# advimman/lama

Hardware: NVIDIA H100
Metric: images/sec FFCResNetGenerator @512x512 bs32 (higher is better)
Workload: dtype bf16x3(f32 accumulate)

## Files before the change

### lama_b200/csrc/conv_tc.cu

```cuda
#include <cuda.h>
#include <stdlib.h>

#include <type_traits>

#include "common.cuh"

namespace ffcb {
namespace {

constexpr int BM = 128;
constexpr int BK = 64;
constexpr int WG_K = 16;
constexpr int kThreads = 384;
constexpr int kConsumers = 256;
constexpr int kTileABytes = BM * BK * 2;
constexpr int kMaxStages = 8;
constexpr int kBarBytes = 1024;
constexpr int kSmemLimit = 227 * 1024;

struct TcParams {
  View out, addend;
  const float* shift;
  int N, act, addend_post;
  int BN, num_n_tiles;
  long long num_m_tiles;
  int stages;
  int flat;
  int TW, TH, tiles_x, tiles_y;
  int stride;
  int coord_off[2];
  int nseg;
  int a_il[2];
  const unsigned short* a_ptr[2];
  long long a_sg[2], a_lo[2];
  int a_tiles_per_image[2];
  int out_planar;
  int ring;
  int hints;
  int rr_dy0, rr_a_bytes, rr_w_bytes;
  int halo_a_bytes;
  signed char seg_taps[FFCB_MAX_KSEG];
  ffcb_kseg seg[FFCB_MAX_KSEG];
};

__device__ __forceinline__ uint32_t smem_u32(const void* p) { return (uint32_t)__cvta_generic_to_shared(p); }

__device__ __forceinline__ void mbar_init(uint64_t* bar, uint32_t count) {
  asm volatile("mbarrier.init.shared::cta.b64 [%0], %1;" ::"r"(smem_u32(bar)), "r"(count));
}
__device__ __forceinline__ void mbar_expect_tx(uint64_t* bar, uint32_t bytes) {
  asm volatile("mbarrier.arrive.expect_tx.shared::cta.b64 _, [%0], %1;" ::"r"(smem_u32(bar)), "r"(bytes) : "memory");
}
__device__ __forceinline__ void mbar_arrive(uint64_t* bar) {
  asm volatile("mbarrier.arrive.shared::cta.b64 _, [%0];" ::"r"(smem_u32(bar)) : "memory");
}
__device__ __forceinline__ void mbar_wait(uint64_t* bar, uint32_t parity) {
  asm volatile(
      "{\n\t"
      ".reg .pred p;\n\t"
      "WAIT_LOOP:\n\t"
      "mbarrier.try_wait.parity.shared::cta.b64 p, [%0], %1;\n\t"
      "@p bra WAIT_DONE;\n\t"
      "bra WAIT_LOOP;\n\t"
      "WAIT_DONE:\n\t"
      "}\n" ::"r"(smem_u32(bar)), "r"(parity)
      : "memory");
}

__device__ __forceinline__ void tma_load_3d(void* dst, const CUtensorMap* map, uint64_t* bar, int c0, int c1, int c2) {
  asm volatile(
      "cp.async.bulk.tensor.3d.shared::cluster.global.mbarrier::complete_tx::bytes [%0], [%1, {%3, %4, %5}], [%2];"
      ::"r"(smem_u32(dst)), "l"(map), "r"(smem_u32(bar)), "r"(c0), "r"(c1), "r"(c2)
      : "memory");
}
__device__ __forceinline__ void tma_load_5d(void* dst, const CUtensorMap* map, uint64_t* bar, int c0, int c1, int c2,
                                            int c3, int c4) {
  asm volatile(
      "cp.async.bulk.tensor.5d.shared::cluster.global.mbarrier::complete_tx::bytes [%0], [%1, {%3, %4, %5, %6, %7}], [%2];"
      ::"r"(smem_u32(dst)), "l"(map), "r"(smem_u32(bar)), "r"(c0), "r"(c1), "r"(c2), "r"(c3), "r"(c4)
      : "memory");
}

__device__ __forceinline__ void bulk_load(void* dst, const void* src, uint32_t bytes, uint64_t* bar) {
  asm volatile("cp.async.bulk.shared::cluster.global.mbarrier::complete_tx::bytes [%0], [%1], %2, [%3];"
               ::"r"(smem_u32(dst)), "l"(src), "r"(bytes), "r"(smem_u32(bar)) : "memory");
}

__device__ __forceinline__ void prefetch_tmap(const CUtensorMap* map) {
  asm volatile("prefetch.tensormap [%0];" ::"l"(map) : "memory");
}

constexpr uint32_t kLoSw = 1u << 16;
constexpr uint32_t kHiSw = (uint32_t)(1024 >> 4) | (1u << 30);
constexpr uint32_t kLoIl = (uint32_t)(2048 >> 4) << 16;
constexpr uint32_t kHiIl = (uint32_t)(128 >> 4);

__device__ __forceinline__ uint32_t desc_addr(uint32_t saddr) { return (saddr & 0x3FFFF) >> 4; }

__device__ __forceinline__ uint64_t desc64(uint32_t lo, uint32_t hi) {
  uint64_t d;
  asm("mov.b64 %0, {%1, %2};" : "=l"(d) : "r"(lo), "r"(hi));
  return d;
}
__device__ __forceinline__ bool elect_one() {
  uint32_t pred;
  asm volatile(
      "{\n\t"
      ".reg .pred P;\n\t"
      "elect.sync _|P, 0xffffffff;\n\t"
      "selp.b32 %0, 1, 0, P;\n\t"
      "}\n"
      : "=r"(pred));
  return pred != 0;
}

__device__ __forceinline__ void wgmma_fence() { asm volatile("wgmma.fence.sync.aligned;" ::: "memory"); }
__device__ __forceinline__ void wgmma_commit() { asm volatile("wgmma.commit_group.sync.aligned;" ::: "memory"); }
template <int N>
__device__ __forceinline__ void wgmma_wait() { asm volatile("wgmma.wait_group.sync.aligned %0;" ::"n"(N) : "memory"); }
template <int BN>
__device__ __forceinline__ void fence_acc(float* d) {
#pragma unroll
  for (int i = 0; i < BN / 2; ++i) asm volatile("" : "+f"(d[i])::"memory");
}

__device__ __forceinline__ void wgmma_n32(float* d, uint64_t da, uint64_t db, uint32_t scale_d) {
  asm volatile(
      "{\n\t.reg .pred p;\n\tsetp.ne.b32 p, %18, 0;\n\t"
      "wgmma.mma_async.sync.aligned.m64n32k16.f32.bf16.bf16 {"
      "%0, %1, %2, %3, %4, %5, %6, %7, %8, %9, %10, %11, %12, %13, %14, %15"
      "}, %16, %17, p, 1, 1, 0, 0;\n\t}\n"
      : "+f"(d[0]), "+f"(d[1]), "+f"(d[2]), "+f"(d[3]), "+f"(d[4]), "+f"(d[5]), "+f"(d[6]), "+f"(d[7]),
        "+f"(d[8]), "+f"(d[9]), "+f"(d[10]), "+f"(d[11]), "+f"(d[12]), "+f"(d[13]), "+f"(d[14]), "+f"(d[15])
      : "l"(da), "l"(db), "r"(scale_d));
}
__device__ __forceinline__ void wgmma_n64(float* d, uint64_t da, uint64_t db, uint32_t scale_d) {
  asm volatile(
      "{\n\t.reg .pred p;\n\tsetp.ne.b32 p, %34, 0;\n\t"
      "wgmma.mma_async.sync.aligned.m64n64k16.f32.bf16.bf16 {"
      "%0, %1, %2, %3, %4, %5, %6, %7, %8, %9, %10, %11, %12, %13, %14, %15, "
      "%16, %17, %18, %19, %20, %21, %22, %23, %24, %25, %26, %27, %28, %29, %30, %31"
      "}, %32, %33, p, 1, 1, 0, 0;\n\t}\n"
      : "+f"(d[0]), "+f"(d[1]), "+f"(d[2]), "+f"(d[3]), "+f"(d[4]), "+f"(d[5]), "+f"(d[6]), "+f"(d[7]),
        "+f"(d[8]), "+f"(d[9]), "+f"(d[10]), "+f"(d[11]), "+f"(d[12]), "+f"(d[13]), "+f"(d[14]), "+f"(d[15]),
        "+f"(d[16]), "+f"(d[17]), "+f"(d[18]), "+f"(d[19]), "+f"(d[20]), "+f"(d[21]), "+f"(d[22]), "+f"(d[23]),
        "+f"(d[24]), "+f"(d[25]), "+f"(d[26]), "+f"(d[27]), "+f"(d[28]), "+f"(d[29]), "+f"(d[30]), "+f"(d[31])
      : "l"(da), "l"(db), "r"(scale_d));
}
__device__ __forceinline__ void wgmma_n96(float* d, uint64_t da, uint64_t db, uint32_t scale_d) {
  asm volatile(
      "{\n\t.reg .pred p;\n\tsetp.ne.b32 p, %50, 0;\n\t"
      "wgmma.mma_async.sync.aligned.m64n96k16.f32.bf16.bf16 {"
      "%0, %1, %2, %3, %4, %5, %6, %7, %8, %9, %10, %11, %12, %13, %14, %15, "
      "%16, %17, %18, %19, %20, %21, %22, %23, %24, %25, %26, %27, %28, %29, %30, %31, "
      "%32, %33, %34, %35, %36, %37, %38, %39, %40, %41, %42, %43, %44, %45, %46, %47"
      "}, %48, %49, p, 1, 1, 0, 0;\n\t}\n"
      : "+f"(d[0]), "+f"(d[1]), "+f"(d[2]), "+f"(d[3]), "+f"(d[4]), "+f"(d[5]), "+f"(d[6]), "+f"(d[7]),
        "+f"(d[8]), "+f"(d[9]), "+f"(d[10]), "+f"(d[11]), "+f"(d[12]), "+f"(d[13]), "+f"(d[14]), "+f"(d[15]),
        "+f"(d[16]), "+f"(d[17]), "+f"(d[18]), "+f"(d[19]), "+f"(d[20]), "+f"(d[21]), "+f"(d[22]), "+f"(d[23]),
        "+f"(d[24]), "+f"(d[25]), "+f"(d[26]), "+f"(d[27]), "+f"(d[28]), "+f"(d[29]), "+f"(d[30]), "+f"(d[31]),
        "+f"(d[32]), "+f"(d[33]), "+f"(d[34]), "+f"(d[35]), "+f"(d[36]), "+f"(d[37]), "+f"(d[38]), "+f"(d[39]),
        "+f"(d[40]), "+f"(d[41]), "+f"(d[42]), "+f"(d[43]), "+f"(d[44]), "+f"(d[45]), "+f"(d[46]), "+f"(d[47])
      : "l"(da), "l"(db), "r"(scale_d));
}
__device__ __forceinline__ void wgmma_n128(float* d, uint64_t da, uint64_t db, uint32_t scale_d) {
  asm volatile(
      "{\n\t.reg .pred p;\n\tsetp.ne.b32 p, %66, 0;\n\t"
      "wgmma.mma_async.sync.aligned.m64n128k16.f32.bf16.bf16 {"
      "%0, %1, %2, %3, %4, %5, %6, %7, %8, %9, %10, %11, %12, %13, %14, %15, "
      "%16, %17, %18, %19, %20, %21, %22, %23, %24, %25, %26, %27, %28, %29, %30, %31, "
      "%32, %33, %34, %35, %36, %37, %38, %39, %40, %41, %42, %43, %44, %45, %46, %47, "
      "%48, %49, %50, %51, %52, %53, %54, %55, %56, %57, %58, %59, %60, %61, %62, %63"
      "}, %64, %65, p, 1, 1, 0, 0;\n\t}\n"
      : "+f"(d[0]), "+f"(d[1]), "+f"(d[2]), "+f"(d[3]), "+f"(d[4]), "+f"(d[5]), "+f"(d[6]), "+f"(d[7]),
        "+f"(d[8]), "+f"(d[9]), "+f"(d[10]), "+f"(d[11]), "+f"(d[12]), "+f"(d[13]), "+f"(d[14]), "+f"(d[15]),
        "+f"(d[16]), "+f"(d[17]), "+f"(d[18]), "+f"(d[19]), "+f"(d[20]), "+f"(d[21]), "+f"(d[22]), "+f"(d[23]),
        "+f"(d[24]), "+f"(d[25]), "+f"(d[26]), "+f"(d[27]), "+f"(d[28]), "+f"(d[29]), "+f"(d[30]), "+f"(d[31]),
        "+f"(d[32]), "+f"(d[33]), "+f"(d[34]), "+f"(d[35]), "+f"(d[36]), "+f"(d[37]), "+f"(d[38]), "+f"(d[39]),
        "+f"(d[40]), "+f"(d[41]), "+f"(d[42]), "+f"(d[43]), "+f"(d[44]), "+f"(d[45]), "+f"(d[46]), "+f"(d[47]),
        "+f"(d[48]), "+f"(d[49]), "+f"(d[50]), "+f"(d[51]), "+f"(d[52]), "+f"(d[53]), "+f"(d[54]), "+f"(d[55]),
        "+f"(d[56]), "+f"(d[57]), "+f"(d[58]), "+f"(d[59]), "+f"(d[60]), "+f"(d[61]), "+f"(d[62]), "+f"(d[63])
      : "l"(da), "l"(db), "r"(scale_d));
}
template <int BN>
__device__ __forceinline__ void wgmma_bn(float* d, uint64_t da, uint64_t db, uint32_t scale_d) {
  static_assert(BN == 32 || BN == 64 || BN == 96 || BN == 128, "N tile");
  if constexpr (BN == 32) wgmma_n32(d, da, db, scale_d);
  else if constexpr (BN == 64) wgmma_n64(d, da, db, scale_d);
  else if constexpr (BN == 96) wgmma_n96(d, da, db, scale_d);
  else wgmma_n128(d, da, db, scale_d);
}

struct TileCoord {
  int b, y0, x0;
  long long m0;
};

__device__ __forceinline__ TileCoord tile_coord(const TcParams& p, long long m_tile) {
  TileCoord t;
  if (p.flat) {
    t.m0 = m_tile * BM;
    t.b = 0; t.y0 = 0; t.x0 = 0;
  } else {
    const int per_img = p.tiles_x * p.tiles_y;
    t.b = (int)(m_tile / per_img);
    const int r = (int)(m_tile - (long long)t.b * per_img);
    t.y0 = (r / p.tiles_x) * p.TH;
    t.x0 = (r % p.tiles_x) * p.TW;
    t.m0 = 0;
  }
  return t;
}

template <bool IL, bool PO, bool RR, bool HALO, int BN>
__global__ void __launch_bounds__(kThreads, 1)
conv_tc_kernel(const __grid_constant__ TcParams p, const __grid_constant__ CUtensorMap map_in0,
               const __grid_constant__ CUtensorMap map_in1, const __grid_constant__ CUtensorMap map_w) {
  extern __shared__ __align__(1024) uint8_t smem_raw[];
  uint8_t* smem = reinterpret_cast<uint8_t*>((reinterpret_cast<uintptr_t>(smem_raw) + 1023) & ~(uintptr_t)1023);
  const int w_bytes = p.BN * BK * 2;
  const int stage_bytes = RR ? 2 * p.rr_a_bytes : HALO ? 2 * w_bytes : 2 * kTileABytes + 2 * w_bytes;
  uint8_t* w_res = smem;
  uint8_t* a_buf = smem;
  if constexpr (RR) smem += p.rr_w_bytes;
  if constexpr (HALO) smem += (size_t)4 * p.halo_a_bytes;
  uint64_t* bars = reinterpret_cast<uint64_t*>(smem + (size_t)p.stages * stage_bytes);
  uint64_t* full = bars;
  uint64_t* empty = bars + kMaxStages;
  uint64_t* w_bar = bars + 2 * kMaxStages;
  uint64_t* a_full = bars + 2 * kMaxStages + 1;
  uint64_t* a_empty = a_full + 2;

  const int warp = threadIdx.x >> 5, lane = threadIdx.x & 31;

  if (warp == 0 && lane == 0) {
    prefetch_tmap(&map_in0);
    prefetch_tmap(&map_in1);
    prefetch_tmap(&map_w);
  }
  if (warp == 1 && lane == 0) {
    for (int s = 0; s < p.stages; ++s) { mbar_init(&full[s], 1); mbar_init(&empty[s], kConsumers); }
    if constexpr (RR) mbar_init(w_bar, 1);
    if constexpr (HALO)
      for (int s = 0; s < 2; ++s) { mbar_init(&a_full[s], 1); mbar_init(&a_empty[s], kConsumers); }
    asm volatile("fence.mbarrier_init.release.cluster;" ::: "memory");
  }
  __syncthreads();

  int total_kblocks = 0;
  for (int s = 0; s < p.nseg; ++s) total_kblocks += (p.seg[s].nch + BK - 1) / BK;
  const long long num_tiles = p.num_m_tiles * p.num_n_tiles;

  if (warp == 0) {
    if constexpr (HALO) {
      int stage = 0, ast = 0;
      uint32_t phase = 0, aph = 0;
      for (long long t = blockIdx.x; t < num_tiles; t += gridDim.x) {
        const int n_tile = (int)(t % p.num_n_tiles);
        const TileCoord tc = tile_coord(p, t / p.num_n_tiles);
        int kofs = 0;
        for (int s = 0; s < p.nseg;) {
          const int ntap = p.seg_taps[s];
          const ffcb_kseg g = p.seg[s];
          const CUtensorMap* map = g.src ? &map_in1 : &map_in0;
          const int nblk = (g.nch + BK - 1) / BK;
          for (int j = 0; j < nblk; ++j) {
            for (int u = 0; u < (ntap == 9 ? 3 : 1); ++u) {
              const int dxu = ntap == 9 ? u - 1 : g.dx;
              mbar_wait(&a_empty[ast], aph ^ 1);
              if (elect_one()) {
                uint8_t* ab = a_buf + (size_t)ast * 2 * p.halo_a_bytes;
                mbar_expect_tx(&a_full[ast], 2u * p.TW * (p.TH + 2) * BK * 2);
                const int cx = tc.x0 + dxu + p.coord_off[g.src], cy = tc.y0 - 1 + p.coord_off[g.src];
                tma_load_5d(ab, map, &a_full[ast], g.c0 + j * BK, cx, cy, tc.b, 0);
                tma_load_5d(ab + p.halo_a_bytes, map, &a_full[ast], g.c0 + j * BK, cx, cy, tc.b, 1);
              }
              __syncwarp();
              if (++ast == 2) { ast = 0; aph ^= 1; }
              for (int tap = 0; tap < ntap; ++tap) {
                if (p.seg[s + tap].dx != dxu) continue;
                mbar_wait(&empty[stage], phase ^ 1);
                if (elect_one()) {
                  uint8_t* st = smem + (size_t)stage * stage_bytes;
                  mbar_expect_tx(&full[stage], (uint32_t)stage_bytes);
                  const int k = kofs + (tap * nblk + j) * BK;
                  tma_load_3d(st, &map_w, &full[stage], k, n_tile * p.BN, 0);
                  tma_load_3d(st + w_bytes, &map_w, &full[stage], k, n_tile * p.BN, 1);
                }
                __syncwarp();
                if (++stage == p.stages) { stage = 0; phase ^= 1; }
              }
            }
          }
          kofs += ntap * nblk * BK;
          s += ntap;
        }
      }
    } else if constexpr (RR) {
      const ffcb_kseg g0 = p.seg[0];
      const CUtensorMap* map = g0.src ? &map_in1 : &map_in0;
      if (elect_one()) {
        mbar_expect_tx(w_bar, (uint32_t)p.rr_w_bytes);
        for (int s = 0; s < p.nseg; ++s) {
          tma_load_3d(w_res + (size_t)s * 2 * w_bytes, &map_w, w_bar, s * BK, 0, 0);
          tma_load_3d(w_res + (size_t)s * 2 * w_bytes + w_bytes, &map_w, w_bar, s * BK, 0, 1);
        }
      }
      __syncwarp();
      int stage = 0;
      uint32_t phase = 0;
      for (long long t = blockIdx.x; t < num_tiles; t += gridDim.x) {
        const TileCoord tc = tile_coord(p, t);
        mbar_wait(&empty[stage], phase ^ 1);
        if (elect_one()) {
          uint8_t* st = smem + (size_t)stage * stage_bytes;
          mbar_expect_tx(&full[stage], (uint32_t)stage_bytes);
          const int cx = tc.x0 + g0.dx + p.coord_off[g0.src], cy = tc.y0 + p.rr_dy0 + p.coord_off[g0.src];
          tma_load_5d(st, map, &full[stage], g0.c0, cx, cy, tc.b, 0);
          tma_load_5d(st + p.rr_a_bytes, map, &full[stage], g0.c0, cx, cy, tc.b, 1);
        }
        __syncwarp();
        if (++stage == p.stages) { stage = 0; phase ^= 1; }
      }
    } else {
      int stage = 0;
      uint32_t phase = 0;
      for (long long t = blockIdx.x; t < num_tiles; t += gridDim.x) {
        const int n_tile = (int)(t % p.num_n_tiles);
        const TileCoord tc = tile_coord(p, t / p.num_n_tiles);
        int kb = 0;
        for (int s = 0; s < p.nseg; ++s) {
          const ffcb_kseg g = p.seg[s];
          const CUtensorMap* map = g.src ? &map_in1 : &map_in0;
          const int nblk = (g.nch + BK - 1) / BK;
          const int cx = tc.x0 * p.stride + g.dx + p.coord_off[g.src];
          const int cy = tc.y0 * p.stride + g.dy + p.coord_off[g.src];
          const int il = IL ? p.a_il[g.src] : 0;
          for (int j = 0; j < nblk; ++j, ++kb) {
            mbar_wait(&empty[stage], phase ^ 1);
            if (elect_one()) {
              uint8_t* st = smem + (size_t)stage * stage_bytes;
              mbar_expect_tx(&full[stage], (uint32_t)stage_bytes);
              const int cc = g.c0 + j * BK;
              if (IL && il) {
                const long long blk = p.flat ? (tc.m0 >> 7)
                                             : (long long)tc.b * p.a_tiles_per_image[g.src] + ((tc.y0 * p.out.W) >> 7);
                const unsigned short* src = p.a_ptr[g.src] + blk * p.a_sg[g.src] + (long long)(cc >> 3) * 1024;
                bulk_load(st, src, kTileABytes, &full[stage]);
                bulk_load(st + kTileABytes, src + p.a_lo[g.src], kTileABytes, &full[stage]);
              } else if (p.flat) {
                tma_load_3d(st, map, &full[stage], cc, (int)tc.m0, 0);
                tma_load_3d(st + kTileABytes, map, &full[stage], cc, (int)tc.m0, 1);
              } else {
                tma_load_5d(st, map, &full[stage], cc, cx, cy, tc.b, 0);
                tma_load_5d(st + kTileABytes, map, &full[stage], cc, cx, cy, tc.b, 1);
              }
              tma_load_3d(st + 2 * kTileABytes, &map_w, &full[stage], kb * BK, n_tile * p.BN, 0);
              tma_load_3d(st + 2 * kTileABytes + w_bytes, &map_w, &full[stage], kb * BK, n_tile * p.BN, 1);
            }
            __syncwarp();
            if (++stage == p.stages) { stage = 0; phase ^= 1; }
          }
        }
      }
    }
  } else if (warp >= 4) {
    const int g = (warp >> 2) - 1;
    const int w = warp & 3, q = lane & 3;
    const int row = g * 64 + w * 16 + (lane >> 2) + 8 * (q & 1);
    const int cb = 4 * (q >> 1);
    const bool odd = (q & 1) != 0;
    const uint32_t a_row_sw = (uint32_t)(g * 64 * BK * 2) >> 4;
    const uint32_t a_row_il = (uint32_t)(g * 64 * 16) >> 4;
    const int HW = p.out.H * p.out.W;
    const bool has_add = p.addend.ptr != nullptr;
    float acc[BN / 2];
#pragma unroll
    for (int i = 0; i < BN / 2; ++i) acc[i] = 0.f;
    int stage = 0, ast = 0;
    uint32_t phase = 0, aph = 0;
    const int a_row0 = (g + 1) * p.TW;
    if constexpr (RR) mbar_wait(w_bar, 0);
    for (long long t = blockIdx.x; t < num_tiles; t += gridDim.x) {
      const int n_tile = (int)(t % p.num_n_tiles);
      const TileCoord tc = tile_coord(p, t / p.num_n_tiles);
      fence_acc<BN>(acc);
      if constexpr (HALO) {
        int prev = -1, a_prev = -1, nt = 0;
        for (int s = 0; s < p.nseg;) {
          const int ntap = p.seg_taps[s];
          const int nblk = (p.seg[s].nch + BK - 1) / BK;
          for (int j = 0; j < nblk; ++j) {
            for (int u = 0; u < (ntap == 9 ? 3 : 1); ++u) {
              const int dxu = ntap == 9 ? u - 1 : p.seg[s].dx;
              mbar_wait(&a_full[ast], aph);
              const uint32_t ab = smem_u32(a_buf + (size_t)ast * 2 * p.halo_a_bytes);
              for (int tap = 0; tap < ntap; ++tap) {
                const int dy = p.seg[s + tap].dy;
                if (p.seg[s + tap].dx != dxu) continue;
                const uint32_t a_off = (uint32_t)((a_row0 + dy * p.TW) * (BK * 2)) >> 4;
                const uint32_t a_hi = desc_addr(ab) + a_off;
                const uint32_t a_lo = desc_addr(ab + (uint32_t)p.halo_a_bytes) + a_off;
                mbar_wait(&full[stage], phase);
                wgmma_fence();
                const uint32_t st = smem_u32(smem + (size_t)stage * stage_bytes);
                const uint32_t w_hi = desc_addr(st), w_lo = desc_addr(st + (uint32_t)w_bytes);
#pragma unroll
                for (int k = 0; k < BK / WG_K; ++k) {
                  const uint32_t adv = (uint32_t)((k * WG_K * 2) >> 4);
                  wgmma_bn<BN>(acc, desc64((a_hi + adv) | kLoSw, kHiSw), desc64((w_hi + adv) | kLoSw, kHiSw),
                               (nt | k) != 0);
                  wgmma_bn<BN>(acc, desc64((a_lo + adv) | kLoSw, kHiSw), desc64((w_hi + adv) | kLoSw, kHiSw), 1);
                  wgmma_bn<BN>(acc, desc64((a_hi + adv) | kLoSw, kHiSw), desc64((w_lo + adv) | kLoSw, kHiSw), 1);
                }
                wgmma_commit();
                wgmma_wait<1>();
                if (prev >= 0) mbar_arrive(&empty[prev]);
                prev = stage;
                if (++stage == p.stages) { stage = 0; phase ^= 1; }
                if (a_prev >= 0) { mbar_arrive(&a_empty[a_prev]); a_prev = -1; }
                ++nt;
              }
              a_prev = ast;
              if (++ast == 2) { ast = 0; aph ^= 1; }
            }
          }
          s += ntap;
        }
        wgmma_wait<0>();
        fence_acc<BN>(acc);
        mbar_arrive(&empty[prev]);
        mbar_arrive(&a_empty[a_prev]);
      } else if constexpr (RR) {
        mbar_wait(&full[stage], phase);
        const uint32_t st = smem_u32(smem + (size_t)stage * stage_bytes);
        const uint32_t wr = smem_u32(w_res);
        for (int sgi = 0; sgi < p.nseg; ++sgi) {
          wgmma_fence();
          const uint32_t a_off = (uint32_t)((p.seg[sgi].dy - p.rr_dy0) * p.TW * (BK * 2));
          const uint32_t a_hi = desc_addr(st + a_off) + a_row_sw;
          const uint32_t a_lo = desc_addr(st + a_off + (uint32_t)p.rr_a_bytes) + a_row_sw;
          const uint32_t w_hi = desc_addr(wr + (uint32_t)(sgi * 2 * w_bytes));
          const uint32_t w_lo = desc_addr(wr + (uint32_t)(sgi * 2 * w_bytes + w_bytes));
#pragma unroll
          for (int k = 0; k < BK / WG_K; ++k) {
            const uint32_t adv = (uint32_t)((k * WG_K * 2) >> 4);
            wgmma_bn<BN>(acc, desc64((a_hi + adv) | kLoSw, kHiSw), desc64((w_hi + adv) | kLoSw, kHiSw), (sgi | k) != 0);
            wgmma_bn<BN>(acc, desc64((a_lo + adv) | kLoSw, kHiSw), desc64((w_hi + adv) | kLoSw, kHiSw), 1);
            wgmma_bn<BN>(acc, desc64((a_hi + adv) | kLoSw, kHiSw), desc64((w_lo + adv) | kLoSw, kHiSw), 1);
          }
          wgmma_commit();
          wgmma_wait<1>();
        }
        wgmma_wait<0>();
        fence_acc<BN>(acc);
        mbar_arrive(&empty[stage]);
        if (++stage == p.stages) { stage = 0; phase ^= 1; }
      } else {
        int prev = -1, sgi = 0, j = 0;
        for (int kb = 0; kb < total_kblocks; ++kb) {
          const bool il = IL && p.a_il[p.seg[sgi].src] != 0;
          const uint32_t a_lodesc = il ? kLoIl : kLoSw, a_hidesc = il ? kHiIl : kHiSw;
          const uint32_t a_row = il ? a_row_il : a_row_sw;
          const uint32_t a_step = il ? (uint32_t)(4096 >> 4) : (uint32_t)((WG_K * 2) >> 4);
          if (IL && ++j == (p.seg[sgi].nch + BK - 1) / BK) { ++sgi; j = 0; }
          mbar_wait(&full[stage], phase);
          wgmma_fence();
          const uint32_t st = smem_u32(smem + (size_t)stage * stage_bytes);
          const uint32_t a_hi = desc_addr(st) + a_row;
          const uint32_t a_lo = desc_addr(st + kTileABytes) + a_row;
          const uint32_t w_hi = desc_addr(st + 2 * kTileABytes);
          const uint32_t w_lo = desc_addr(st + 2 * kTileABytes + w_bytes);
#pragma unroll
          for (int k = 0; k < BK / WG_K; ++k) {
            const uint32_t wadv = (uint32_t)((k * WG_K * 2) >> 4);
            const uint32_t aadv = (uint32_t)k * a_step;
            wgmma_bn<BN>(acc, desc64((a_hi + aadv) | a_lodesc, a_hidesc), desc64((w_hi + wadv) | kLoSw, kHiSw),
                         (kb | k) != 0);
            wgmma_bn<BN>(acc, desc64((a_lo + aadv) | a_lodesc, a_hidesc), desc64((w_hi + wadv) | kLoSw, kHiSw), 1);
            wgmma_bn<BN>(acc, desc64((a_hi + aadv) | a_lodesc, a_hidesc), desc64((w_lo + wadv) | kLoSw, kHiSw), 1);
          }
          wgmma_commit();
          wgmma_wait<1>();
          if (prev >= 0) mbar_arrive(&empty[prev]);
          prev = stage;
          if (++stage == p.stages) { stage = 0; phase ^= 1; }
        }
        wgmma_wait<0>();
        fence_acc<BN>(acc);
        mbar_arrive(&empty[prev]);
      }

      int b, y, x;
      bool valid;
      if (p.flat) {
        const unsigned m = (unsigned)tc.m0 + (unsigned)row;
        valid = m < (unsigned)(p.out.B * HW);
        const unsigned mm = valid ? m : 0u;
        b = (int)(mm / (unsigned)HW);
        const unsigned r = mm - (unsigned)b * (unsigned)HW;
        y = (int)(r / (unsigned)p.out.W);
        x = (int)(r - (unsigned)y * (unsigned)p.out.W);
      } else {
        b = tc.b;
        y = tc.y0 + row / p.TW;
        x = tc.x0 + row % p.TW;
        valid = y < p.out.H && x < p.out.W;
      }
      const long long o_out = valid ? pix_off(p.out, b, y, x) : 0;
      const long long o_add = (has_add && valid) ? pix_off(p.addend, b, y, x) : 0;
      int mir_dy = 0, mir_dx = 0;
      if (!PO && p.ring && valid) {
        int my, mx;
        if (ring_mirrors(p.out, y, x, my, mx)) {
          if (my != -2) mir_dy = (my - y) * (int)p.out.sy;
          if (mx != -2) mir_dx = (mx - x) * (int)p.out.sx;
        }
      }
      const uint64_t pol = l2_policy(PO && p.hints ? 2 : 0);
#pragma unroll
      for (int j = 0; j < BN / 8; ++j) {
        const float s0 = odd ? acc[4 * j] : acc[4 * j + 2], s1 = odd ? acc[4 * j + 1] : acc[4 * j + 3];
        const float r0 = __shfl_xor_sync(0xffffffffu, s0, 1), r1 = __shfl_xor_sync(0xffffffffu, s1, 1);
        float4 v = odd ? make_float4(r0, r1, acc[4 * j + 2], acc[4 * j + 3])
                       : make_float4(acc[4 * j], acc[4 * j + 1], r0, r1);
        const int n = n_tile * p.BN + 8 * j + cb;
        if (!valid || n >= p.N) continue;
        if (p.shift != nullptr) {
          const float4 sh = __ldg(reinterpret_cast<const float4*>(p.shift + n));
          v.x += sh.x; v.y += sh.y; v.z += sh.z; v.w += sh.w;
        }
        float4 ad = make_float4(0.f, 0.f, 0.f, 0.f);
        if (has_add) ad = load4(p.addend, o_add + n);
        if (!p.addend_post) { v.x += ad.x; v.y += ad.y; v.z += ad.z; v.w += ad.w; }
        if (p.act == FFCB_ACT_RELU) {
          v.x = fmaxf(v.x, 0.f); v.y = fmaxf(v.y, 0.f); v.z = fmaxf(v.z, 0.f); v.w = fmaxf(v.w, 0.f);
        } else if (p.act != FFCB_ACT_NONE) {
          v.x = slow_act(v.x, p.act); v.y = slow_act(v.y, p.act); v.z = slow_act(v.z, p.act); v.w = slow_act(v.w, p.act);
        }
        if (p.addend_post) { v.x += ad.x; v.y += ad.y; v.z += ad.z; v.w += ad.w; }
        if constexpr (PO) {
          st_hint_f4(reinterpret_cast<float*>(p.out.ptr) + o_out + chan_off(p.out, n), v, pol);
        } else {
          store4(p.out, o_out + n, v);
          if (mir_dy) store4(p.out, o_out + mir_dy + n, v);
          if (mir_dx) store4(p.out, o_out + mir_dx + n, v);
          if (mir_dy && mir_dx) store4(p.out, o_out + mir_dy + mir_dx + n, v);
        }
      }
    }
  }
}

typedef CUresult (*EncodeTiledFn)(CUtensorMap*, CUtensorMapDataType, cuuint32_t, void*, const cuuint64_t*,
                                  const cuuint64_t*, const cuuint32_t*, const cuuint32_t*, CUtensorMapInterleave,
                                  CUtensorMapSwizzle, CUtensorMapL2promotion, CUtensorMapFloatOOBfill);

EncodeTiledFn get_encode() {
  static EncodeTiledFn fn = nullptr;
  if (fn == nullptr) {
    void* p = nullptr;
    cudaDriverEntryPointQueryResult q;
    if (cudaGetDriverEntryPoint("cuTensorMapEncodeTiled", &p, cudaEnableDefault, &q) == cudaSuccess &&
        q == cudaDriverEntryPointSuccess)
      fn = reinterpret_cast<EncodeTiledFn>(p);
  }
  return fn;
}

int encode_typed(CUtensorMap* map, void* base, CUtensorMapDataType dt, CUtensorMapSwizzle sw, int rank,
                 const cuuint64_t* dims, const cuuint64_t* strides_bytes, const cuuint32_t* box, const cuuint32_t* estr,
                 const char* what) {
  EncodeTiledFn fn = get_encode();
  if (fn == nullptr) {
    set_error("conv(tc): cuTensorMapEncodeTiled entry point unavailable");
    return FFCB_ECUDA;
  }
  CUresult r = fn(map, dt, (cuuint32_t)rank, base, dims, strides_bytes, box, estr, CU_TENSOR_MAP_INTERLEAVE_NONE, sw,
                  CU_TENSOR_MAP_L2_PROMOTION_L2_256B, CU_TENSOR_MAP_FLOAT_OOB_FILL_NONE);
  if (r != CUDA_SUCCESS) {
    set_error("conv(tc): cuTensorMapEncodeTiled(%s) failed with CUresult %d (rank %d, dims %llu %llu %llu, box %u %u %u)",
              what, (int)r, rank, (unsigned long long)dims[0], (unsigned long long)dims[1],
              (unsigned long long)(rank > 2 ? dims[2] : 0), box[0], box[1], rank > 2 ? box[2] : 0);
    return FFCB_ECUDA;
  }
  return FFCB_OK;
}

int encode(CUtensorMap* map, void* base, int rank, const cuuint64_t* dims, const cuuint64_t* strides_bytes,
           const cuuint32_t* box, const cuuint32_t* estr, const char* what) {
  return encode_typed(map, base, CU_TENSOR_MAP_DATA_TYPE_BFLOAT16, CU_TENSOR_MAP_SWIZZLE_128B, rank, dims, strides_bytes,
                      box, estr, what);
}

int pick_bn(int n) {
  if (const char* e = getenv("FFCB_TC_BN")) {
    const int v = atoi(e);
    if (v >= 32 && v <= 128 && v % 32 == 0) return v < n ? v : (n + 31) / 32 * 32;
  }
  if (n <= 128) return (n + 31) / 32 * 32;
  if (n == 192) return 96;
  return 128;
}

}

int conv_tc(const ffcb_conv_desc* d, cudaStream_t stream) {
  FFCB_REQUIRE(d->out.B > 0, "conv(tc): empty batch");
  FFCB_REQUIRE((long long)d->out.B * d->out.H * d->out.W < (1ll << 31), "conv(tc): more than 2^31 output pixels");
  bool used[2] = {false, false}, taps[2] = {false, false};
  int reach[2] = {0, 0};
  for (int i = 0; i < d->nseg; ++i) {
    used[d->seg[i].src] = true;
    if (d->seg[i].dx != 0 || d->seg[i].dy != 0) taps[d->seg[i].src] = true;
    const int ax = d->seg[i].dx < 0 ? -d->seg[i].dx : d->seg[i].dx, ay = d->seg[i].dy < 0 ? -d->seg[i].dy : d->seg[i].dy;
    if (ax > reach[d->seg[i].src]) reach[d->seg[i].src] = ax;
    if (ay > reach[d->seg[i].src]) reach[d->seg[i].src] = ay;
    FFCB_REQUIRE(d->seg[i].c0 % 8 == 0, "conv(tc): segment %d starts at channel %d (must be a multiple of 8)", i,
                 d->seg[i].c0);
  }
  for (int s = 0; s < 2; ++s) {
    if (!used[s]) continue;
    const ffcb_tensor& t = d->in[s];
    FFCB_REQUIRE(t.fmt == FFCB_BF16X2, "conv(tc): in[%d] must be split bf16 (FFCB_BF16X2)", s);
    if (t.cg != 0) {
      FFCB_REQUIRE(t.cg == 8 && t.tile == 128 && !taps[s] && d->stride == 1 && t.H == d->out.H && t.W == d->out.W,
                   "conv(tc): a channel-group planar in[%d] must be tile-blocked (tile=128, cg=8) with 1x1 taps, stride 1",
                   s);
      for (int i = 0; i < d->nseg; ++i)
        if (d->seg[i].src == s)
          FFCB_REQUIRE(d->seg[i].nch % 64 == 0 && d->seg[i].c0 % 8 == 0,
                       "conv(tc): segment %d of a channel-group planar input must cover whole 64-channel blocks", i);
    }
    FFCB_REQUIRE(t.sx % 8 == 0 && t.sy % 8 == 0 && t.sb % 8 == 0 && t.lo_off % 8 == 0 && ((uintptr_t)t.ptr % 16) == 0,
                 "conv(tc): in[%d] strides / pointer not 16-byte aligned", s);
    if (taps[s] && d->border == FFCB_BORDER_REFLECT)
      FFCB_REQUIRE(t.pad >= reach[s] && t.reflect_border, "conv(tc): in[%d] needs a reflected border ring of %d pixels",
                   s, reach[s]);
  }

  TcParams p;
  p.out = make_view(d->out);
  p.out_planar = d->out.cg != 0 ? 1 : 0;
  p.ring = (d->out.reflect_border && d->out.pad == 1 && d->out.cg == 0 && d->out.fmt == FFCB_BF16X2 && d->out.H >= 4 &&
            d->out.W >= 4) ? 1 : 0;
  if (d->out.cg != 0)
    FFCB_REQUIRE(d->out.fmt == FFCB_F32 && d->out.sx % 4 == 0 && d->out.sy % 4 == 0 && d->out.sb % 4 == 0,
                 "conv(tc): channel-group planar outputs are float32");
  if (d->out.cg != 0)
    FFCB_REQUIRE(d->out.sg % 4 == 0 && (reinterpret_cast<uintptr_t>(d->out.ptr) & 15) == 0,
                 "conv(tc): planar output needs 16-byte aligned channel groups");
  p.hints = l2_hints_enabled() ? 1 : 0;
  p.addend = d->addend.ptr ? make_view(d->addend) : null_view();
  p.shift = d->shift;
  p.N = d->n_out; p.act = d->act; p.addend_post = d->addend_post;
  p.BN = pick_bn(d->n_out);
  p.num_n_tiles = (d->n_out + p.BN - 1) / p.BN;
  p.stride = d->stride;
  p.nseg = d->nseg;
  int kpad = 0;
  for (int i = 0; i < d->nseg; ++i) {
    p.seg[i] = d->seg[i];
    kpad += (d->seg[i].nch + BK - 1) / BK * BK;
  }

  const int H = d->out.H, W = d->out.W;
  bool flat = d->stride == 1 && !taps[0] && !taps[1];
  for (int s = 0; s < 2 && flat; ++s) {
    if (!used[s]) continue;
    const ffcb_tensor& t = d->in[s];
    flat = t.H == H && t.W == W && (t.tile != 0 || (t.sy == (int64_t)W * t.sx && t.sb == (int64_t)H * t.sy));
  }
  for (int s = 0; s < 2; ++s) {
    p.a_il[s] = 0; p.a_ptr[s] = nullptr; p.a_sg[s] = p.a_lo[s] = 0; p.a_tiles_per_image[s] = 0;
    if (!used[s] || d->in[s].cg == 0) continue;
    const ffcb_tensor& t = d->in[s];
    p.a_il[s] = 1;
    p.a_ptr[s] = reinterpret_cast<const unsigned short*>(t.ptr);
    p.a_sg[s] = t.sg; p.a_lo[s] = t.lo_off;
    p.a_tiles_per_image[s] = (t.H * t.W) >> 7;
    FFCB_REQUIRE(t.lo_off % 8 == 0, "conv(tc): tile-blocked in[%d]: lo plane not 16-byte aligned", s);
  }
  p.flat = flat ? 1 : 0;
  bool rr = false;
  int rr_dy_min = 0, rr_dy_max = 0;
  p.rr_dy0 = p.rr_a_bytes = p.rr_w_bytes = 0;
  {
    const char* e = getenv("FFCB_TC_ROWS");
    rr = !flat && d->stride == 1 && d->nseg >= 3 && p.num_n_tiles == 1 && (e ? atoi(e) != 0 : true) &&
         d->in[d->seg[0].src].cg == 0;
    rr_dy_min = rr_dy_max = d->seg[0].dy;
    for (int i = 0; i < d->nseg && rr; ++i) {
      const ffcb_kseg& g = d->seg[i];
      rr = g.src == d->seg[0].src && g.c0 == d->seg[0].c0 && g.nch == BK && g.dx == d->seg[0].dx;
      for (int j = 0; j < i && rr; ++j) rr = d->seg[j].dy != g.dy;
      if (g.dy < rr_dy_min) rr_dy_min = g.dy;
      if (g.dy > rr_dy_max) rr_dy_max = g.dy;
    }
    rr = rr && (rr_dy_max - rr_dy_min) <= 8;
  }
  bool halo = !flat && !rr && d->stride == 1 && W > 32 && d->out.cg == 0;
  int ngroups = 0;
  for (int i = 0; i < d->nseg && halo;) {
    const ffcb_kseg& g = d->seg[i];
    const ffcb_tensor& t = d->in[g.src];
    halo = t.cg == 0 && d->border == FFCB_BORDER_REFLECT && taps[g.src] && t.pad >= 1 && t.window == 0;
    unsigned mask = 0;
    int n = 0;
    for (; n < 9 && i + n < d->nseg; ++n) {
      const ffcb_kseg& q = d->seg[i + n];
      if (q.src != g.src || q.c0 != g.c0 || q.nch != g.nch || q.dy < -1 || q.dy > 1 || q.dx < -1 || q.dx > 1) break;
      mask |= 1u << ((q.dy + 1) * 3 + q.dx + 1);
    }
    if (n == 9 && mask == 0x1FFu) {
      p.seg_taps[i] = 9;
      for (int k = 1; k < 9; ++k) p.seg_taps[i + k] = 0;
      i += 9;
      ++ngroups;
    } else {
      halo = halo && g.dy >= -1 && g.dy <= 1 && g.dx >= -1 && g.dx <= 1;
      p.seg_taps[i++] = 1;
    }
  }
  halo = halo && ngroups > 0;
  p.halo_a_bytes = 0;
  if (flat) {
    p.TW = BM; p.TH = 1; p.tiles_x = p.tiles_y = 1;
    p.num_m_tiles = ((long long)d->out.B * H * W + BM - 1) / BM;
  } else if (rr) {
    const char* etw = getenv("FFCB_TC_ROWS_TW");
    p.TW = (etw && atoi(etw) == 16) ? 16 : 8;
    p.TH = BM / p.TW;
    p.tiles_x = (W + p.TW - 1) / p.TW;
    p.tiles_y = (H + p.TH - 1) / p.TH;
    p.num_m_tiles = (long long)d->out.B * p.tiles_x * p.tiles_y;
    p.rr_dy0 = rr_dy_min;
    p.rr_a_bytes = (p.TH + rr_dy_max - rr_dy_min) * p.TW * BK * 2;
    p.rr_w_bytes = d->nseg * 2 * p.BN * BK * 2;
  } else if (halo) {
    p.TW = 64; p.TH = 2;
    p.tiles_x = (W + p.TW - 1) / p.TW;
    p.tiles_y = (H + p.TH - 1) / p.TH;
    p.num_m_tiles = (long long)d->out.B * p.tiles_x * p.tiles_y;
    p.halo_a_bytes = p.TW * (p.TH + 2) * BK * 2;
  } else {
    int tw = 1;
    while (tw < W && tw < BM) tw <<= 1;
    p.TW = tw; p.TH = BM / tw;
    p.tiles_x = (W + p.TW - 1) / p.TW;
    p.tiles_y = (H + p.TH - 1) / p.TH;
    p.num_m_tiles = (long long)d->out.B * p.tiles_x * p.tiles_y;
    FFCB_REQUIRE(p.TW * d->stride <= 256 && p.TH * d->stride <= 256, "conv(tc): tile exceeds the TMA box limit");
  }

  for (int s = 0; s < 2; ++s)
    if (p.a_il[s] && !flat)
      FFCB_REQUIRE(p.TW == W && p.TW * p.TH == BM && H % p.TH == 0 && (H * W) % BM == 0,
                   "conv(tc): tile-blocked in[%d] in a spatial contraction needs M tiles of whole rows (W a power of two "
                   "<= 128 dividing 128, H*W a multiple of 128); got %dx%d", s, H, W);

  alignas(64) CUtensorMap maps[3];
  int rc;
  for (int s = 0; s < 2; ++s) {
    if (!used[s]) { p.coord_off[s] = 0; continue; }
    const ffcb_tensor& t = d->in[s];
    const cuuint64_t esz = 2;
    if (p.a_il[s]) { p.coord_off[s] = 0; continue; }
    if (flat) {
      cuuint64_t dims[3] = {(cuuint64_t)t.C, (cuuint64_t)t.B * t.H * t.W, 2};
      cuuint64_t str[2] = {(cuuint64_t)t.sx * esz, (cuuint64_t)t.lo_off * esz};
      cuuint32_t box[3] = {BK, BM, 1}, es[3] = {1, 1, 1};
      p.coord_off[s] = 0;
      if ((rc = encode(&maps[s], t.ptr, 3, dims, str, box, es, "flat activations"))) return rc;
    } else {
      const bool ring = taps[s] && d->border == FFCB_BORDER_REFLECT;
      const int off = ring ? t.pad : 0;
      char* base = (char*)t.ptr - (int64_t)off * ((int64_t)t.sy + t.sx) * (int64_t)esz;
      cuuint64_t dims[5] = {(cuuint64_t)t.C, (cuuint64_t)(t.W + 2 * off), (cuuint64_t)(t.H + 2 * off),
                            (cuuint64_t)t.B, 2};
      cuuint64_t str[4] = {(cuuint64_t)t.sx * esz, (cuuint64_t)t.sy * esz, (cuuint64_t)t.sb * esz,
                           (cuuint64_t)t.lo_off * esz};
      cuuint32_t box[5] = {BK, (cuuint32_t)(p.TW * d->stride), (cuuint32_t)(p.TH * d->stride), 1, 1};
      if (rr) box[2] = (cuuint32_t)(p.TH + rr_dy_max - rr_dy_min);
      if (halo) box[2] = (cuuint32_t)(p.TH + 2);
      cuuint32_t es[5] = {1, (cuuint32_t)d->stride, (cuuint32_t)d->stride, 1, 1};
      p.coord_off[s] = off;
      if ((rc = encode(&maps[s], base, 5, dims, str, box, es, "spatial activations"))) return rc;
    }
  }
  {
    cuuint64_t dims[3] = {(cuuint64_t)kpad, (cuuint64_t)d->n_out, 2};
    cuuint64_t str[2] = {(cuuint64_t)kpad * 2, (cuuint64_t)kpad * d->n_out * 2};
    cuuint32_t box[3] = {BK, (cuuint32_t)p.BN, 1}, es[3] = {1, 1, 1};
    FFCB_REQUIRE(((uintptr_t)d->weight % 16) == 0, "conv(tc): weight pointer not 16-byte aligned");
    if ((rc = encode(&maps[2], const_cast<void*>(d->weight), 3, dims, str, box, es, "weights"))) return rc;
  }

  for (int s = 0; s < 2; ++s)
    if (!used[s] || p.a_il[s]) maps[s] = maps[2];
  if (d->out.cg == 0) {
    const ffcb_tensor& t = d->out;
    const cuuint64_t esz = t.fmt == FFCB_BF16X2 ? 2 : 4;
    FFCB_REQUIRE(((uintptr_t)t.ptr % 16) == 0 && (t.sx * esz) % 16 == 0 && (t.sy * esz) % 16 == 0 &&
                     (t.sb * esz) % 16 == 0 && (esz == 4 || (t.lo_off * esz) % 16 == 0),
                 "conv(tc): out strides / pointer not 16-byte aligned (C must be a multiple of %d)", esz == 2 ? 8 : 4);
  }

  const int stage_bytes = rr ? 2 * p.rr_a_bytes : halo ? 2 * p.BN * BK * 2 : 2 * kTileABytes + 2 * p.BN * BK * 2;
  const int bar_bytes = kBarBytes + (rr ? p.rr_w_bytes : 0) + (halo ? 4 * p.halo_a_bytes : 0);
  int stages = (kSmemLimit - 1024 - bar_bytes) / stage_bytes;
  if (stages > kMaxStages) stages = kMaxStages;
  FFCB_REQUIRE(stages >= 2, "conv(tc): BN=%d leaves fewer than 2 pipeline stages", p.BN);
  p.stages = stages;
  const size_t smem = (size_t)stages * stage_bytes + bar_bytes + 1024;
  int dev = 0, sms = 132;
  FFCB_CUDA(cudaGetDevice(&dev));
  FFCB_CUDA(cudaDeviceGetAttribute(&sms, cudaDevAttrMultiProcessorCount, dev));
  const long long tiles = p.num_m_tiles * p.num_n_tiles;
  const int grid = (int)(tiles < sms ? tiles : sms);
  const bool any_il = p.a_il[0] || p.a_il[1];
  auto launch = [&](auto kernel) -> int {
    FFCB_CUDA(cudaFuncSetAttribute(kernel, cudaFuncAttributeMaxDynamicSharedMemorySize, kSmemLimit));
    kernel<<<grid, kThreads, smem, stream>>>(p, maps[0], maps[1], maps[2]);
    return FFCB_OK;
  };
  auto launch_bn = [&](auto bn) -> int {
    constexpr int N = decltype(bn)::value;
    if (rr) return launch(conv_tc_kernel<false, false, true, false, N>);
    if (halo) return launch(conv_tc_kernel<false, false, false, true, N>);
    if (any_il)
      return p.out_planar ? launch(conv_tc_kernel<true, true, false, false, N>)
                          : launch(conv_tc_kernel<true, false, false, false, N>);
    return p.out_planar ? launch(conv_tc_kernel<false, true, false, false, N>)
                        : launch(conv_tc_kernel<false, false, false, false, N>);
  };
  switch (p.BN) {
    case 32: rc = launch_bn(std::integral_constant<int, 32>()); break;
    case 64: rc = launch_bn(std::integral_constant<int, 64>()); break;
    case 96: rc = launch_bn(std::integral_constant<int, 96>()); break;
    default: rc = launch_bn(std::integral_constant<int, 128>()); break;
  }
  if (rc) return rc;
  FFCB_LAUNCH_CHECK("conv_tc_kernel");
  return FFCB_OK;
}

}
```

Baseline: 316.8.

## Pair CTAs in clusters and multicast weight tiles via TMA

Launches the tensor-core conv kernel as 2-CTA clusters when there are enough K blocks. Each CTA of a pair loads half of each weight stage with TMA multicast, so both CTAs receive the full weight tile while global/L2 weight traffic is cut roughly in half. Stage release now has one arrive per consumer warp on both the local and the peer empty barrier, and cluster syncs are added at start and end. The cost is cross-CTA coupling, since a pair stalls together, plus padded dummy tiles when the M-tile count is odd and a possibly smaller grid set by cluster occupancy.

```diff
diff --git a/lama_b200/csrc/conv_tc.cu b/lama_b200/csrc/conv_tc.cu
--- a/lama_b200/csrc/conv_tc.cu
+++ b/lama_b200/csrc/conv_tc.cu
@@ -67,10 +67,32 @@
       : "memory");
 }
 
+__device__ __forceinline__ void mbar_arrive_rank(uint64_t* bar, uint32_t rank) {
+  uint32_t remote;
+  asm volatile("mapa.shared::cluster.u32 %0, %1, %2;" : "=r"(remote) : "r"(smem_u32(bar)), "r"(rank));
+  asm volatile("mbarrier.arrive.shared::cluster.b64 _, [%0];" ::"r"(remote) : "memory");
+}
+__device__ __forceinline__ uint32_t cluster_ctarank() {
+  uint32_t r;
+  asm volatile("mov.u32 %0, %%cluster_ctarank;" : "=r"(r));
+  return r;
+}
+__device__ __forceinline__ void cluster_sync() {
+  asm volatile("barrier.cluster.arrive.release;\n\tbarrier.cluster.wait.acquire;" ::: "memory");
+}
+
 __device__ __forceinline__ void tma_load_3d(void* dst, const CUtensorMap* map, uint64_t* bar, int c0, int c1, int c2) {
   asm volatile(
       "cp.async.bulk.tensor.3d.shared::cluster.global.mbarrier::complete_tx::bytes [%0], [%1, {%3, %4, %5}], [%2];"
       ::"r"(smem_u32(dst)), "l"(map), "r"(smem_u32(bar)), "r"(c0), "r"(c1), "r"(c2)
+      : "memory");
+}
+__device__ __forceinline__ void tma_load_3d_mc(void* dst, const CUtensorMap* map, uint64_t* bar, int c0, int c1, int c2,
+                                               uint16_t mask) {
+  asm volatile(
+      "cp.async.bulk.tensor.3d.shared::cluster.global.mbarrier::complete_tx::bytes.multicast::cluster"
+      " [%0], [%1, {%3, %4, %5}], [%2], %6;"
+      ::"r"(smem_u32(dst)), "l"(map), "r"(smem_u32(bar)), "r"(c0), "r"(c1), "r"(c2), "h"(mask)
       : "memory");
 }
 __device__ __forceinline__ void tma_load_5d(void* dst, const CUtensorMap* map, uint64_t* bar, int c0, int c1, int c2,
@@ -212,7 +234,40 @@
   return t;
 }
 
-template <bool IL, bool PO, bool RR, bool HALO, int BN>
+struct Unit {
+  int n_tile;
+  long long m_tile;
+  bool store;
+};
+__device__ __forceinline__ Unit unit_tile(const TcParams& p, long long u, uint32_t rank, int cl) {
+  Unit r;
+  r.n_tile = (int)(u % p.num_n_tiles);
+  r.m_tile = (u / p.num_n_tiles) * cl + rank;
+  r.store = r.m_tile < p.num_m_tiles;
+  if (!r.store) r.m_tile = p.num_m_tiles - 1;
+  return r;
+}
+
+__device__ __forceinline__ void load_weights(uint8_t* w, int w_bytes, const CUtensorMap* map, uint64_t* bar, int k, int n0,
+                                             int cl, uint32_t rank) {
+  if (cl == 1) {
+    tma_load_3d(w, map, bar, k, n0, 0);
+    tma_load_3d(w + w_bytes, map, bar, k, n0, 1);
+  } else {
+    tma_load_3d_mc(w + rank * w_bytes, map, bar, k, n0, (int)rank, (uint16_t)0x3);
+  }
+}
+
+__device__ __forceinline__ void release_stage(uint64_t* bar, int cl, uint32_t rank, int lane) {
+  if (cl == 1) {
+    mbar_arrive(bar);
+  } else if (lane == 0) {
+    mbar_arrive(bar);
+    mbar_arrive_rank(bar, rank ^ 1);
+  }
+}
+
+template <bool IL, bool PO, bool RR, bool HALO, bool PAIR, int BN>
 __global__ void __launch_bounds__(kThreads, 1)
 conv_tc_kernel(const __grid_constant__ TcParams p, const __grid_constant__ CUtensorMap map_in0,
                const __grid_constant__ CUtensorMap map_in1, const __grid_constant__ CUtensorMap map_w) {
@@ -232,6 +287,8 @@
   uint64_t* a_empty = a_full + 2;
 
   const int warp = threadIdx.x >> 5, lane = threadIdx.x & 31;
+  constexpr int cl = PAIR ? 2 : 1;
+  const uint32_t rank = PAIR ? cluster_ctarank() : 0u;
 
   if (warp == 0 && lane == 0) {
     prefetch_tmap(&map_in0);
@@ -239,25 +296,31 @@
     prefetch_tmap(&map_w);
   }
   if (warp == 1 && lane == 0) {
-    for (int s = 0; s < p.stages; ++s) { mbar_init(&full[s], 1); mbar_init(&empty[s], kConsumers); }
+    for (int s = 0; s < p.stages; ++s) {
+      mbar_init(&full[s], 1);
+      mbar_init(&empty[s], PAIR ? (kConsumers / 32) * cl : kConsumers);
+    }
     if constexpr (RR) mbar_init(w_bar, 1);
     if constexpr (HALO)
       for (int s = 0; s < 2; ++s) { mbar_init(&a_full[s], 1); mbar_init(&a_empty[s], kConsumers); }
     asm volatile("fence.mbarrier_init.release.cluster;" ::: "memory");
   }
-  __syncthreads();
+  if constexpr (PAIR) cluster_sync();
+  else __syncthreads();
 
   int total_kblocks = 0;
   for (int s = 0; s < p.nseg; ++s) total_kblocks += (p.seg[s].nch + BK - 1) / BK;
-  const long long num_tiles = p.num_m_tiles * p.num_n_tiles;
+  const long long num_units = (p.num_m_tiles + cl - 1) / cl * p.num_n_tiles;
+  const long long u0 = blockIdx.x / cl, du = gridDim.x / cl;
 
   if (warp == 0) {
     if constexpr (HALO) {
       int stage = 0, ast = 0;
       uint32_t phase = 0, aph = 0;
-      for (long long t = blockIdx.x; t < num_tiles; t += gridDim.x) {
-        const int n_tile = (int)(t % p.num_n_tiles);
-        const TileCoord tc = tile_coord(p, t / p.num_n_tiles);
+      for (long long u = u0; u < num_units; u += du) {
+        const Unit un = unit_tile(p, u, rank, cl);
+        const int n_tile = un.n_tile;
+        const TileCoord tc = tile_coord(p, un.m_tile);
         int kofs = 0;
         for (int s = 0; s < p.nseg;) {
           const int ntap = p.seg_taps[s];
@@ -284,8 +347,7 @@
                   uint8_t* st = smem + (size_t)stage * stage_bytes;
                   mbar_expect_tx(&full[stage], (uint32_t)stage_bytes);
                   const int k = kofs + (tap * nblk + j) * BK;
-                  tma_load_3d(st, &map_w, &full[stage], k, n_tile * p.BN, 0);
-                  tma_load_3d(st + w_bytes, &map_w, &full[stage], k, n_tile * p.BN, 1);
+                  load_weights(st, w_bytes, &map_w, &full[stage], k, n_tile * p.BN, cl, rank);
                 }
                 __syncwarp();
                 if (++stage == p.stages) { stage = 0; phase ^= 1; }
@@ -309,8 +371,8 @@
       __syncwarp();
       int stage = 0;
       uint32_t phase = 0;
-      for (long long t = blockIdx.x; t < num_tiles; t += gridDim.x) {
-        const TileCoord tc = tile_coord(p, t);
+      for (long long u = u0; u < num_units; u += du) {
+        const TileCoord tc = tile_coord(p, u);
         mbar_wait(&empty[stage], phase ^ 1);
         if (elect_one()) {
           uint8_t* st = smem + (size_t)stage * stage_bytes;
@@ -325,9 +387,10 @@
     } else {
       int stage = 0;
       uint32_t phase = 0;
-      for (long long t = blockIdx.x; t < num_tiles; t += gridDim.x) {
-        const int n_tile = (int)(t % p.num_n_tiles);
-        const TileCoord tc = tile_coord(p, t / p.num_n_tiles);
+      for (long long u = u0; u < num_units; u += du) {
+        const Unit un = unit_tile(p, u, rank, cl);
+        const int n_tile = un.n_tile;
+        const TileCoord tc = tile_coord(p, un.m_tile);
         int kb = 0;
         for (int s = 0; s < p.nseg; ++s) {
           const ffcb_kseg g = p.seg[s];
@@ -355,8 +418,7 @@
                 tma_load_5d(st, map, &full[stage], cc, cx, cy, tc.b, 0);
                 tma_load_5d(st + kTileABytes, map, &full[stage], cc, cx, cy, tc.b, 1);
               }
-              tma_load_3d(st + 2 * kTileABytes, &map_w, &full[stage], kb * BK, n_tile * p.BN, 0);
-              tma_load_3d(st + 2 * kTileABytes + w_bytes, &map_w, &full[stage], kb * BK, n_tile * p.BN, 1);
+              load_weights(st + 2 * kTileABytes, w_bytes, &map_w, &full[stage], kb * BK, n_tile * p.BN, cl, rank);
             }
             __syncwarp();
             if (++stage == p.stages) { stage = 0; phase ^= 1; }
@@ -381,9 +443,10 @@
     uint32_t phase = 0, aph = 0;
     const int a_row0 = (g + 1) * p.TW;
     if constexpr (RR) mbar_wait(w_bar, 0);
-    for (long long t = blockIdx.x; t < num_tiles; t += gridDim.x) {
-      const int n_tile = (int)(t % p.num_n_tiles);
-      const TileCoord tc = tile_coord(p, t / p.num_n_tiles);
+    for (long long u = u0; u < num_units; u += du) {
+      const Unit un = unit_tile(p, u, rank, cl);
+      const int n_tile = un.n_tile;
+      const TileCoord tc = tile_coord(p, un.m_tile);
       fence_acc<BN>(acc);
       if constexpr (HALO) {
         int prev = -1, a_prev = -1, nt = 0;
@@ -415,7 +478,7 @@
                 }
                 wgmma_commit();
                 wgmma_wait<1>();
-                if (prev >= 0) mbar_arrive(&empty[prev]);
+                if (prev >= 0) release_stage(&empty[prev], cl, rank, lane);
                 prev = stage;
                 if (++stage == p.stages) { stage = 0; phase ^= 1; }
                 if (a_prev >= 0) { mbar_arrive(&a_empty[a_prev]); a_prev = -1; }
@@ -429,7 +492,7 @@
         }
         wgmma_wait<0>();
         fence_acc<BN>(acc);
-        mbar_arrive(&empty[prev]);
+        release_stage(&empty[prev], cl, rank, lane);
         mbar_arrive(&a_empty[a_prev]);
       } else if constexpr (RR) {
         mbar_wait(&full[stage], phase);
@@ -454,7 +517,7 @@
         }
         wgmma_wait<0>();
         fence_acc<BN>(acc);
-        mbar_arrive(&empty[stage]);
+        release_stage(&empty[stage], cl, rank, lane);
         if (++stage == p.stages) { stage = 0; phase ^= 1; }
       } else {
         int prev = -1, sgi = 0, j = 0;
@@ -482,20 +545,21 @@
           }
           wgmma_commit();
           wgmma_wait<1>();
-          if (prev >= 0) mbar_arrive(&empty[prev]);
+          if (prev >= 0) release_stage(&empty[prev], cl, rank, lane);
           prev = stage;
           if (++stage == p.stages) { stage = 0; phase ^= 1; }
         }
         wgmma_wait<0>();
         fence_acc<BN>(acc);
-        mbar_arrive(&empty[prev]);
+        release_stage(&empty[prev], cl, rank, lane);
       }
 
+      const bool store = un.store;
       int b, y, x;
       bool valid;
       if (p.flat) {
         const unsigned m = (unsigned)tc.m0 + (unsigned)row;
-        valid = m < (unsigned)(p.out.B * HW);
+        valid = store && m < (unsigned)(p.out.B * HW);
         const unsigned mm = valid ? m : 0u;
         b = (int)(mm / (unsigned)HW);
         const unsigned r = mm - (unsigned)b * (unsigned)HW;
@@ -505,7 +569,7 @@
         b = tc.b;
         y = tc.y0 + row / p.TW;
         x = tc.x0 + row % p.TW;
-        valid = y < p.out.H && x < p.out.W;
+        valid = store && y < p.out.H && x < p.out.W;
       }
       const long long o_out = valid ? pix_off(p.out, b, y, x) : 0;
       const long long o_add = (has_add && valid) ? pix_off(p.addend, b, y, x) : 0;
@@ -550,6 +614,7 @@
       }
     }
   }
+  if constexpr (PAIR) cluster_sync();
 }
 
 typedef CUresult (*EncodeTiledFn)(CUtensorMap*, CUtensorMapDataType, cuuint32_t, void*, const cuuint64_t*,
@@ -816,23 +881,49 @@
   int dev = 0, sms = 132;
   FFCB_CUDA(cudaGetDevice(&dev));
   FFCB_CUDA(cudaDeviceGetAttribute(&sms, cudaDevAttrMultiProcessorCount, dev));
-  const long long tiles = p.num_m_tiles * p.num_n_tiles;
-  const int grid = (int)(tiles < sms ? tiles : sms);
+  bool pair = !rr && !halo && p.num_m_tiles >= 2 && kpad / BK >= 8;
+  if (const char* e = getenv("FFCB_TC_MULTICAST")) pair = !rr && p.num_m_tiles >= 2 && atoi(e) != 0;
+  const int cluster = pair ? 2 : 1;
+  const long long units = (p.num_m_tiles + cluster - 1) / cluster * p.num_n_tiles;
   const bool any_il = p.a_il[0] || p.a_il[1];
   auto launch = [&](auto kernel) -> int {
     FFCB_CUDA(cudaFuncSetAttribute(kernel, cudaFuncAttributeMaxDynamicSharedMemorySize, kSmemLimit));
-    kernel<<<grid, kThreads, smem, stream>>>(p, maps[0], maps[1], maps[2]);
+    cudaLaunchAttribute attr;
+    attr.id = cudaLaunchAttributeClusterDimension;
+    attr.val.clusterDim.x = (unsigned)cluster;
+    attr.val.clusterDim.y = 1;
+    attr.val.clusterDim.z = 1;
+    cudaLaunchConfig_t cfg = {};
+    cfg.blockDim = dim3(kThreads);
+    cfg.dynamicSmemBytes = smem;
+    cfg.stream = stream;
+    cfg.attrs = &attr;
+    cfg.numAttrs = cluster > 1 ? 1 : 0;
+    int slots = sms;
+    if (cluster > 1) {
+      cfg.gridDim = dim3((unsigned)(2 * sms));
+      FFCB_CUDA(cudaOccupancyMaxActiveClusters(&slots, kernel, &cfg));
+      FFCB_REQUIRE(slots > 0, "conv(tc): no CTA pair of %zu bytes of shared memory fits on the device", smem);
+    }
+    const long long grid = units < slots ? units : slots;
+    cfg.gridDim = dim3((unsigned)(grid * cluster));
+    FFCB_CUDA(cudaLaunchKernelEx(&cfg, kernel, p, maps[0], maps[1], maps[2]));
     return FFCB_OK;
+  };
+  auto launch_mode = [&](auto bn, auto pr) -> int {
+    constexpr int N = decltype(bn)::value;
+    constexpr bool PR = decltype(pr)::value;
+    if (halo) return launch(conv_tc_kernel<false, false, false, true, PR, N>);
+    if (any_il)
+      return p.out_planar ? launch(conv_tc_kernel<true, true, false, false, PR, N>)
+                          : launch(conv_tc_kernel<true, false, false, false, PR, N>);
+    return p.out_planar ? launch(conv_tc_kernel<false, true, false, false, PR, N>)
+                        : launch(conv_tc_kernel<false, false, false, false, PR, N>);
   };
   auto launch_bn = [&](auto bn) -> int {
     constexpr int N = decltype(bn)::value;
-    if (rr) return launch(conv_tc_kernel<false, false, true, false, N>);
-    if (halo) return launch(conv_tc_kernel<false, false, false, true, N>);
-    if (any_il)
-      return p.out_planar ? launch(conv_tc_kernel<true, true, false, false, N>)
-                          : launch(conv_tc_kernel<true, false, false, false, N>);
-    return p.out_planar ? launch(conv_tc_kernel<false, true, false, false, N>)
-                        : launch(conv_tc_kernel<false, false, false, false, N>);
+    if (rr) return launch(conv_tc_kernel<false, false, true, false, false, N>);
+    return pair ? launch_mode(bn, std::true_type()) : launch_mode(bn, std::false_type());
   };
   switch (p.BN) {
     case 32: rc = launch_bn(std::integral_constant<int, 32>()); break;
```

Measured after the change: 315.6 (median of 6 runs). Within noise of the previous version (-0.4%).
